# halismai/photobundle

Hardware: AMD Instinct MI355X
Metric: LM iters/sec + residuals/sec, 8-frame KITTI window, 50k pts, 5x5 patch (higher is better)
Workload: dtype f64; 1 GPU; configs[1]: 8-frame window, 50000 points/GPU, 5x5 patch, single level, dense visibility; image=1241x376 u8, observations=400000, sampler_precision=exact, channels=1, point_parameterisation=free world points (reference)

## Files before the change

__graft_entry__.py:

```python
import os
import subprocess
import sys

ROOT = os.path.dirname(os.path.abspath(__file__))
if ROOT not in sys.path:
    sys.path.insert(0, ROOT)


def build():
    env = dict(os.environ)
    subprocess.check_call(["make", "-s", "-C", os.path.join(ROOT, "photobundle_amd", "csrc")], env=env)
    subprocess.check_call(["make", "-s", "-C", os.path.join(ROOT, "photobundle_amd", "host")], env=env)
    subprocess.check_call(["make", "-s", "-C", os.path.join(ROOT, "oracle")], env=env)
    subprocess.check_call(["make", "-s", "-C", os.path.join(ROOT, "tests", "native")], env=env)
    import photobundle_amd
    from photobundle_amd import _lib
    _lib.lib()


def smoke():
    import numpy as np
    from oracle import oracle
    from photobundle_amd import synthetic
    from photobundle_amd.engine import Engine, default_solver_options

    p = synthetic.make_window(n_frames=4, n_points=300, radius=2, size=(120, 160), K=(200.0, 200.0, 80.0, 60.0))
    ref = oracle.solve(p, oracle.default_options(max_num_iterations=8))
    with Engine(120, 160, p.K, p.radius, p.n_frames, huber=p.huber, device=0) as e:
        e.load(p)
        res = e.solve(default_solver_options(max_num_iterations=8))
    assert len(res["iterations"]) == len(ref["iterations"])
    for a, b in zip(ref["iterations"], res["iterations"]):
        assert a["step_is_successful"] == b["step_is_successful"]
        assert abs(a["cost"] - b["cost"]) <= 1e-9 * abs(a["cost"]), (a["cost"], b["cost"])
    err = float(np.abs(res["cams"] - ref["cams"]).max())
    assert err <= 1e-5, err
    print("smoke ok: final cost %.6e (oracle %.6e), max pose diff %.3e" % (res["final_cost"], ref["final_cost"], err))


if __name__ == "__main__":
    build()
    if len(sys.argv) > 1 and sys.argv[1] == "smoke":
        smoke()
```

photobundle_amd/csrc/pba_solve.h:

```cpp
#pragma once

namespace pba {

__host__ __device__ inline int tri_index(int r) { return r * (r + 1) / 2; }
__host__ __device__ inline int packed_stride(int n) { return tri_index(n + 1) + 2 * n + 2; }

__host__ __device__ inline int solve_item_base(int j, int N1) { return (j - 1) * (N1 - 3 * j); }
inline int solve_table_words(int nf) { const int n = 6 * nf; return tri_index(n + 1) + (nf > 1 ? solve_item_base(nf, n + 1) : 0); }
inline void solve_tables(int nf, uint32_t* tab) {
  const int n = 6 * nf, N1 = n + 1, TRI = tri_index(N1);
  for (int r = 0; r < N1; ++r)
    for (int c = 0; c <= r; ++c) tab[tri_index(r) + c] = ((uint32_t)r << 16) | (uint32_t)c;
  for (int j = 1; j < nf; ++j)
    for (int r = 6 * j; r <= n; ++r) tab[TRI + solve_item_base(j, N1) + (r - 6 * j)] = (uint32_t)r | ((uint32_t)j << 16);
}

__device__ __forceinline__ int packed_dest(int e, int nf, int n_pairs) {
  const int n = 6 * nf, nT = 36 * n_pairs;
  if (e < nT) {
    const int pair = PBA_PARTIAL_T ? e % n_pairs : e / 36, k = PBA_PARTIAL_T ? e / n_pairs : e - 36 * pair, i = k / 6, j = k - 6 * i;
    int a = 0, rem = pair;
    while (rem >= nf - a) { rem -= nf - a; ++a; }
    const int b = a + rem;
    if (a == b && j < i) return -1;
// ... 250 lines not shown
}

__global__ __launch_bounds__(kSolveThreads) void k_solve_generic(SolveParams p_in) {
  SolveParams p = p_in;
  if (!solve_resolve(p)) return;
  extern __shared__ __attribute__((aligned(16))) char smem[];
  const int n = 6 * p.n_free;
  const int ld = n + 1;
  double* S = reinterpret_cast<double*>(smem);
  double* y = S + n * ld;
  double* sc = y + n;
  double* D2 = sc + n;
  double* gcs = D2 + n;
  double* gc = gcs + n;
  __shared__ int s_ok;
  const int tid = threadIdx.x;
  if (tid == 0) s_ok = 1;
  if (p.peer_world > 0 && !peer_wait_all(p.peer, p.peer_world, p.peer_flag, p.peer_seq, p.peer_timeout, p.peer_err, tid)) s_ok = 0;
  solve_prologue<kSolveThreads>(p, n, ld, S, y, sc, D2, gcs, gc, tid);
  const int tx = tid & 15, ty = tid >> 4;
  for (int j = 0; j < n; ++j) {
    const double d = S[j * ld + j];
    const double dj = (d > 0.0) ? sqrt(d) : 1.0;
    if (tid == 0 && (!(d > 0.0) || !isfinite(d))) s_ok = 0;
    __syncthreads();
    for (int r = j + tid; r < n; r += kSolveThreads) S[r * ld + j] = (r == j) ? dj : S[r * ld + j] / dj;
    __syncthreads();
    for (int r = j + 1 + ty; r < n; r += 16) {
      const double lrj = S[r * ld + j];
      for (int c = j + 1 + tx; c <= r; c += 16) S[r * ld + c] -= lrj * S[c * ld + j];
    }
    __syncthreads();
  }
  for (int j = 0; j < n; ++j) {
    if (tid == 0) y[j] /= S[j * ld + j];
    __syncthreads();
    const double yj = y[j];
    for (int r = j + 1 + tid; r < n; r += kSolveThreads) y[r] -= S[r * ld + j] * yj;
    __syncthreads();
  }
  for (int j = n - 1; j >= 0; --j) {
    if (tid == 0) y[j] /= S[j * ld + j];
    __syncthreads();
    const double yj = y[j];
    for (int r = tid; r < j; r += kSolveThreads) y[r] -= S[j * ld + r] * yj;
    __syncthreads();
  }
  solve_epilogue<kSolveThreads>(p, n, y, sc, D2, gcs, gc, s_ok != 0, tid);
}

constexpr int kSolveBlockedThreads = 256;
constexpr int kSolveWideThreads = 512;
constexpr int kSolveNarrowFree = 8;
__host__ __device__ inline size_t solve_blocked_smem_bytes(int n) {
  const size_t N1 = (size_t)n + 1;
  const size_t items = (size_t)(n / 6) * N1;
  return sizeof(double) * (N1 * N1 + 2 * 6 * N1 + 6 * N1 + 2) + sizeof(uint32_t) * items;
}

__device__ inline void cam_geom_scalar(const double cam6[6], double* cg) {
  const double wx = cam6[0], wy = cam6[1], wz = cam6[2];
  const double theta2 = wx * wx + wy * wy + wz * wz;
  const bool rod = theta2 > DBL_EPSILON;
#pragma unroll
  for (int k = 0; k < 6; ++k) cg[k] = cam6[k];
  double R[9], w3[3], ct, st;
  if (rod) {
    const double theta = sqrt(theta2);
    sincos_angle(theta, st, ct);
    const double ti = 1.0 / theta;
    const double ax = wx * ti, ay = wy * ti, az = wz * ti;
    const double oc = 1.0 - ct;
    w3[0] = ax; w3[1] = ay; w3[2] = az;
    R[0] = ct + ax * ax * oc;       R[1] = ax * ay * oc - az * st;  R[2] = ay * st + ax * az * oc;
    R[3] = az * st + ax * ay * oc;  R[4] = ct + ay * ay * oc;       R[5] = -ax * st + ay * az * oc;
    R[6] = -ay * st + ax * az * oc; R[7] = ax * st + ay * az * oc;  R[8] = ct + az * az * oc;
  } else {
    w3[0] = w3[1] = w3[2] = 0.0; ct = 1.0; st = 0.0;
    R[0] = 1; R[1] = -wz; R[2] = wy; R[3] = wz; R[4] = 1; R[5] = -wx; R[6] = -wy; R[7] = wx; R[8] = 1;
  }
#pragma unroll
  for (int k = 0; k < 3; ++k) cg[6 + k] = w3[k];
  cg[9] = ct; cg[10] = st;
#pragma unroll
  for (int k = 0; k < 9; ++k) cg[11 + k] = R[k];
  cg[20] = theta2;
  cg[21] = rod ? 1.0 : 0.0;
}

__device__ inline void cam_geom_finish(const double* cg, CamGeom* __restrict__ out, int c, uint32_t anchor_mask, int sub) {
  CamGeom& g = out[c];
  const bool rod = cg[21] != 0.0;
  if (sub < 3) { g.aa[sub] = cg[sub]; g.t[sub] = cg[3 + sub]; g.w[sub] = cg[6 + sub]; }
  if (sub == 3) {
    g.rodrigues = rod; g.is_free = slot_is_free(anchor_mask, c);
    g.free_index = slot_free_index(anchor_mask, c);
    g.pad = 0;
  }
  if (sub == 4) { g.ct = cg[9]; g.st = cg[10]; }
  const double* R = cg + 11;
  const int e9 = sub < 9 ? sub : 8;
  if (sub < 9) g.R[sub] = R[e9];
  const int s27 = sub < 27 ? sub : 26;
  double dRv;
  if (rod) {
    const int ei = e9 / 3, ej = e9 - 3 * ei;
    double acc = cg[ei] * cg[ej];
#pragma unroll
    for (int q = 0; q < 3; ++q) {
      const int d = (ej - q + 3) % 3;
      const double wo = cg[(d == 0) ? 0 : 3 - q - ej];
      const double wxqj = (d == 0) ? 0.0 : (d == 1 ? -wo : wo);
      acc += (R[3 * q + ei] - (ei == q ? 1.0 : 0.0)) * wxqj;
    }
    const double Bv = acc / cg[20];
    const int k = s27 / 9, ij = s27 - 9 * k, i = ij / 3, j = ij - 3 * i;
    const int lane0 = threadIdx.x & 32;
    const double b0 = __shfl(Bv, lane0 + k), b1 = __shfl(Bv, lane0 + 3 + k), b2 = __shfl(Bv, lane0 + 6 + k);
    const double x0 = (j == 0) ? 0.0 : (j == 1 ? -b2 : b1);
    const double x1 = (j == 0) ? b2 : (j == 1 ? 0.0 : -b0);
    const double x2 = (j == 0) ? -b1 : (j == 1 ? b0 : 0.0);
    double a3 = 0.0;
    a3 += R[3 * i] * x0; a3 += R[3 * i + 1] * x1; a3 += R[3 * i + 2] * x2;
    dRv = a3;
  } else {
    const int k = s27 / 9, m = s27 - 9 * k;
    const int i = m / 3, j = m - 3 * i;
    dRv = 0.0;
    if (i != j && i != k && j != k) dRv = ((j - i + 3) % 3 == 1) ? -1.0 : 1.0;
  }
  if (sub < 27) g.dR[sub] = dRv;
}

template <bool AGENT, int T>
__device__ __forceinline__ void solve_blocked(SolveParams& p, double* smem, int tid) {
  const int nf = p.n_free;
  const int n = 6 * nf;
  const int N1 = n + 1;
  const int ld = N1;
  double* A = smem;
  double* Wp = A + (size_t)N1 * ld;
  double* xs = Wp + 2 * (size_t)N1 * 6;
  double* sc = xs + N1;
  double* D2 = sc + N1;
  double* gcs = D2 + N1;
  double* gc = gcs + N1;
  double* live = gc + N1;
  uint32_t* items = reinterpret_cast<uint32_t*>(live + N1 + 1);
  __shared__ int s_ok;
  __shared__ double s_cams[6 * kMaxFrames];
  __shared__ int s_free[kMaxFrames];
  __shared__ double s_cg[kMaxFrames][32];
  __shared__ double s_stat[3];
  __shared__ double s_dyn[3];
  const int TRI = tri_index(N1);
  const int lane = tid & 63, wave = __builtin_amdgcn_readfirstlane(tid >> 6);
  unsigned long long ts[8] = {0, 0, 0, 0, 0, 0, 0, 0};
#define PBA_TS(k) do { if (PBA_PHASE_TIMING) ts[k] = __builtin_amdgcn_s_memtime(); } while (0)
  unsigned long long sec[8] = {0, 0, 0, 0, 0, 0, 0, 0}, sec_t = 0;
#define PBA_SEC(k) do { if (PBA_PHASE_TIMING) { const unsigned long long tn = __builtin_amdgcn_s_memtime(); if (k) sec[k] += tn - sec_t; sec_t = tn; } } while (0)
  PBA_TS(0);
  bool peer_ok = true;
  if (!AGENT && p.peer_world > 0) peer_ok = peer_wait_all(p.peer, p.peer_world, p.peer_flag, p.peer_seq, p.peer_timeout, p.peer_err, tid);
  constexpr int kPer = (T > 256) ? 9 : 5;
  double val[kPer];
#pragma unroll
  for (int u = 0; u < kPer; ++u) { const int t = tid + u * T; val[u] = (t < TRI) ? packed_load<AGENT>(p, t) : 0.0; }
  const double cam_v = (tid < 6 * p.n_frames) ? p.cams[tid] : 0.0;
  const int free_v = (tid < p.n_frames) ? p.geom[tid].free_index : -1;
  static_assert(T >= 6 * kMaxFrames, "one thread per reduced-system row");
  double du = 0.0, g = 0.0, s_old = 1.0, live_old = 0.0, cost_lin = 0.0, gn2_pts = 0.0;
  if (tid < n) {
    du = packed_load<AGENT>(p, TRI + n + tid);
    g = packed_load<AGENT>(p, TRI + tid);
    if (!p.init_scale) { s_old = p.sc[tid]; live_old = p.sc[n + tid]; }
  }
  if (tid == 0) { cost_lin = packed_load<AGENT>(p, TRI + 2 * n); gn2_pts = packed_load<AGENT>(p, TRI + 2 * n + 1); }
  uint32_t rc[kPer];
#pragma unroll
  for (int u = 0; u < kPer; ++u) { const int t = tid + u * T; rc[u] = (t < TRI) ? p.tab[t] : 0u; }
  const int n_items = (nf > 1) ? solve_item_base(nf, N1) : 0;
  constexpr int kItemsPer = (T > 256) ? 2 : 1;
  uint32_t itv[kItemsPer];
#pragma unroll
  for (int u = 0; u < kItemsPer; ++u) { const int t = tid + u * T; itv[u] = (t < n_items) ? p.tab[TRI + t] : 0u; }
#pragma unroll
  for (int u = 0; u < kItemsPer; ++u) { const int t = tid + u * T; if (t < n_items) items[t] = itv[u]; }
  if (tid < 6 * p.n_frames) s_cams[tid] = cam_v;
  if (tid < p.n_frames) s_free[tid] = free_v;
  if (tid < n) {
    const int i = tid;
    double s, lv;
    if (p.init_scale) { s = p.jacobi ? 1.0 / (1.0 + sqrt(du)) : 1.0; lv = du > 0.0 ? 1.0 : 0.0; p.sc[i] = s; p.sc[n + i] = lv; }
    else { s = s_old; lv = live_old; }
    sc[i] = s;
    live[i] = lv;
    D2[i] = fmin(fmax(s * s * du, p.min_diag), p.max_diag) / p.radius;
    gc[i] = g;
    gcs[i] = s * g;
  }
  if (tid == n) sc[n] = 1.0;
  if (tid == 0) s_ok = peer_ok ? 1 : 0;
  __syncthreads();
  PBA_TS(1);
#pragma unroll
  for (int u = 0; u < kPer; ++u) {
    const int t = tid + u * T;
    if (t >= TRI) continue;
    const int r = (int)(rc[u] >> 16), c = (int)(rc[u] & 0xffffu);
    double v = sc[c] * val[u] * sc[r];
    if (r == c) v = (r < n) ? v + D2[r] : 0.0;
    A[(size_t)r * ld + c] = v;
    if (r != c) A[(size_t)c * ld + r] = 0.0;
  }
  __syncthreads();
  if (p.S_dbg) {
    for (int k = tid; k < n * n; k += T) { const int r = k / n, c = k - r * n; p.S_dbg[k] = (r >= c) ? A[(size_t)r * ld + c] : A[(size_t)c * ld + r]; }
    for (int i = tid; i < n; i += T) p.rhs_dbg[i] = A[(size_t)n * ld + i];
    __syncthreads();
  }
  PBA_TS(2);
  constexpr int ROWS = (T > 256) ? 2 : 1;
  constexpr int NB = T - 64;
  if (wave == T / 64 - 1) {
    double q2[2] = {0.0, 0.0};
    double gmax = 0.0;
    for (int i = lane; i < n; i += 64) { gmax = fmax(gmax, fabs(gc[i])); q2[0] += gc[i] * gc[i]; }
    for (int i = lane; i < 6 * p.n_frames; i += 64) {
      const int fa = s_free[i / 6];
      if (fa < 0) continue;
      const double* lv = live + 6 * fa;
      if (lv[0] + lv[1] + lv[2] + lv[3] + lv[4] + lv[5] > 0.0) q2[1] += s_cams[i] * s_cams[i];
    }
    wave_sum_n<2>(q2);
    gmax = wave_max(gmax);
    if (lane == 0) { s_stat[0] = gmax; s_stat[1] = q2[0]; s_stat[2] = q2[1]; }
  }
  if (!(p.final_pass && !p.init_scale)) {
    if (wave == 0) {
      __builtin_amdgcn_s_setprio(3);
      double a[ROWS][6], w[ROWS][6];
      double Wd[21];
#pragma unroll
      for (int q = 0; q < ROWS; ++q) {
        const int r = lane + 64 * q;
#pragma unroll
        for (int m = 0; m < 6; ++m) { a[q][m] = A[(size_t)(r <= n ? r : n) * ld + m]; w[q][m] = 0.0; }
      }
#pragma unroll
      for (int i = 0; i < 6; ++i)
#pragma unroll
        for (int m = 0; m <= i; ++m) Wd[i * (i + 1) / 2 + m] = A[(size_t)i * ld + m];
      for (int k = 0; k < nf; ++k) {
        const int c0 = 6 * k;
        double Lt[21], rd[6];
        bool pd = true;
        PBA_SEC(0);
#pragma unroll
        for (int j = 0; j < 6; ++j) {
#pragma unroll
          for (int i = j; i < 6; ++i) {
            double v = Wd[i * (i + 1) / 2 + j];
#pragma unroll
            for (int m = 0; m < j; ++m) v = fma(-Wd[i * (i + 1) / 2 + m], Lt[j * (j + 1) / 2 + m], v);
            Wd[i * (i + 1) / 2 + j] = v;
          }
          const double d = Wd[j * (j + 1) / 2 + j];
          const bool ok = (d > 0.0) && isfinite(d);
          pd = pd && ok;
          rd[j] = fast_rcp(ok ? d : 1.0);
#pragma unroll
          for (int i = j + 1; i < 6; ++i) Lt[i * (i + 1) / 2 + j] = Wd[i * (i + 1) / 2 + j] * rd[j];
        }
        PBA_SEC(1);
        double* Wk = Wp + (size_t)(k & 1) * N1 * 6;
#pragma unroll
        for (int q = 0; q < ROWS; ++q) {
          const int r = lane + 64 * q;
          double l[6];
#pragma unroll
          for (int j = 0; j < 6; ++j) {
            double v = a[q][j];
#pragma unroll
            for (int m = 0; m < j; ++m) v = fma(-w[q][m], Lt[j * (j + 1) / 2 + m], v);
            w[q][j] = v;
            l[j] = v * rd[j];
          }
          if (r >= c0 && r <= n) {
#pragma unroll
            for (int m = 0; m < 6; ++m) { A[(size_t)r * ld + c0 + m] = l[m]; Wk[(size_t)r * 6 + m] = w[q][m]; }
            if (r == c0 && !pd) s_ok = 0;
          }
        }
        PBA_SEC(2);
        double Lb[36];
        const bool more = k + 1 < nf;
        if (more) {
          wave_lds_sync();
#pragma unroll
          for (int e = 0; e < 6; ++e)
#pragma unroll
            for (int m = 0; m < 6; ++m) Lb[6 * e + m] = A[(size_t)(c0 + 6 + e) * ld + c0 + m];
        }
        PBA_SEC(3);
        __syncthreads();
        PBA_SEC(4);
        if (!more) break;
#pragma unroll
        for (int q = 0; q < ROWS; ++q) {
          const int r = lane + 64 * q;
          const bool act = r >= c0 + 6 && r <= n;
          const double* arow = A + (size_t)(r <= n ? r : n) * ld + c0 + 6;
          double an[6];
#pragma unroll
          for (int e = 0; e < 6; ++e) an[e] = arow[e];
#pragma unroll
          for (int m = 0; m < 6; ++m)
#pragma unroll
            for (int e = 0; e < 6; ++e) an[e] = fma(-w[q][m], Lb[6 * e + m], an[e]);
          if (act && r < c0 + 12) {
#pragma unroll
            for (int e = 0; e < 6; ++e) A[(size_t)r * ld + c0 + 6 + e] = an[e];
          }
#pragma unroll
          for (int e = 0; e < 6; ++e) a[q][e] = an[e];
        }
        PBA_SEC(5);
        wave_lds_sync();
#pragma unroll
        for (int i = 0; i < 6; ++i)
#pragma unroll
          for (int m = 0; m <= i; ++m) Wd[i * (i + 1) / 2 + m] = A[(size_t)(c0 + 6 + i) * ld + c0 + 6 + m];
        if (PBA_PHASE_TIMING) { asm volatile("s_waitcnt lgkmcnt(0)" ::: "memory"); }
        PBA_SEC(6);
      }
      __builtin_amdgcn_s_setprio(0);
    } else {
      const int qb = tid - 64;
      for (int k = 0; k < nf; ++k) {
        __syncthreads();
        if (k + 2 >= nf) continue;
        const int c0 = 6 * k;
        const double* Wk = Wp + (size_t)(k & 1) * N1 * 6;
        for (int it = solve_item_base(k + 2, N1) + qb; it < n_items; it += NB) {
          const uint32_t wd = items[it];
          const int r = (int)(wd & 0xffffu), j = (int)(wd >> 16);
          double wr[6], lc[36], acc[6];
#pragma unroll
          for (int m = 0; m < 6; ++m) wr[m] = Wk[(size_t)r * 6 + m];
#pragma unroll
          for (int e = 0; e < 6; ++e)
#pragma unroll
            for (int m = 0; m < 6; ++m) lc[6 * e + m] = A[(size_t)(6 * j + e) * ld + c0 + m];
#pragma unroll
          for (int e = 0; e < 6; ++e) acc[e] = A[(size_t)r * ld + 6 * j + e];
#pragma unroll
          for (int e = 0; e < 6; ++e)
#pragma unroll
            for (int m = 0; m < 6; ++m) acc[e] = fma(-wr[m], lc[6 * e + m], acc[e]);
#pragma unroll
          for (int e = 0; e < 6; ++e) A[(size_t)r * ld + 6 * j + e] = acc[e];
        }
      }
    }
    for (int t = tid; t < n; t += T) {
      const int c0 = 6 * (t / 6);
#pragma unroll
      for (int m = 0; m < 6; ++m) if (c0 + m >= t) A[(size_t)t * ld + c0 + m] = 0.0;
    }
    __syncthreads();
    PBA_TS(3);
    if (wave == 0) {
      double z[ROWS];
#pragma unroll
      for (int q = 0; q < ROWS; ++q) { const int i = lane + 64 * q; z[q] = (i < n) ? A[(size_t)n * ld + i] : 0.0; }
      const double* Arow = A + (lane < n ? lane : 0);
      auto load_chunk = [&](int jb, double (&L6)[6][ROWS]) {
#pragma unroll
        for (int u = 0; u < 6; ++u)
#pragma unroll
          for (int q = 0; q < ROWS; ++q) L6[u][q] = Arow[(size_t)(jb + u) * ld + 64 * q];
      };
      auto apply_chunk = [&](int jb, const double (&L6)[6][ROWS]) {
#pragma unroll
        for (int u = 5; u >= 0; --u) {
          const int j = jb + u;
          const double zsrc = (ROWS == 2 && j >= 64) ? z[ROWS - 1] : z[0];
          const double xj = readlane_f64(zsrc, j & 63);
#pragma unroll
          for (int q = 0; q < ROWS; ++q) z[q] = fma(-L6[u][q], xj, z[q]);
        }
      };
      double LA[6][ROWS], LB[6][ROWS];
      int jb = n - 6;
      load_chunk(jb, LA);
      for (;;) {
        if (jb >= 6) load_chunk(jb - 6, LB);
        apply_chunk(jb, LA);
        jb -= 6;
        if (jb < 0) break;
        if (jb >= 6) load_chunk(jb - 6, LA);
        apply_chunk(jb, LB);
        jb -= 6;
        if (jb < 0) break;
      }
      double q2[2] = {0.0, 0.0};
      bool bad = false;
#pragma unroll
      for (int q = 0; q < ROWS; ++q) {
        const int i = lane + 64 * q;
        if (i < n) {
          xs[i] = z[q];
          q2[0] += 0.5 * z[q] * gcs[i] + 0.5 * D2[i] * z[q] * z[q];
          const double d = sc[i] * z[q];
          q2[1] += d * d;
          bad = bad || !isfinite(z[q]);
        }
      }
      wave_sum_n<2>(q2);
      const bool any_bad = __any(bad ? 1 : 0) != 0;
      if (lane == 0) { s_dyn[0] = q2[0]; s_dyn[1] = q2[1]; s_dyn[2] = any_bad ? 1.0 : 0.0; }
    }
    __syncthreads();
  } else {
    for (int i = tid; i < n; i += T) xs[i] = 0.0;
    if (tid == 0) { s_dyn[0] = 0.0; s_dyn[1] = 0.0; s_dyn[2] = 0.0; }
    __syncthreads();
  }
  PBA_TS(4);
  const bool chol_ok = s_ok != 0;
  const bool poisoned = !AGENT && p.peer_world > 0 && !peer_ok;
  const double qnan = __longlong_as_double(0x7ff8000000000000ll);
  if (tid < 6 * p.n_frames && !(p.final_pass && !p.init_scale)) {
    const int slot = tid / 6, k = tid % 6;
    const int fa = s_free[slot];
    double d = 0.0;
    if (fa >= 0) d = -sc[6 * fa + k] * xs[6 * fa + k];
    if (poisoned) d = qnan;
    p.delta_c[tid] = d;
    p.cams_cand[tid] = s_cams[tid] + d;
  }
  if (p.geom_cand) {
    if (wave == 1 && lane < p.n_frames) {
      const int c = lane;
      double cam6[6];
      const int fa = s_free[c];
#pragma unroll
      for (int k = 0; k < 6; ++k) cam6[k] = s_cams[6 * c + k] + (fa >= 0 ? -sc[6 * fa + k] * xs[6 * fa + k] : 0.0);
      cam_geom_scalar(cam6, s_cg[c]);
    }
  }
  if (tid == 0) {
    p.scal[kMccCams] = s_dyn[0]; p.scal[kStep2Cams] = s_dyn[1]; p.scal[kX2Cams] = s_stat[2];
    p.scal[kGmaxCams] = s_stat[0]; p.scal[kGnorm2Cams] = s_stat[1];
    p.scal[kSolveOk] = (chol_ok && s_dyn[2] == 0.0 && !poisoned) ? 1.0 : 0.0;
    p.scal[kCostLin] = poisoned ? qnan : cost_lin;
    p.scal[kGnorm2Pts] = gn2_pts;
  }
  PBA_TS(6);
  if (p.geom_cand) {
    __syncthreads();
    for (int c = tid / 32; c < p.n_frames; c += T / 32) cam_geom_finish(s_cg[c], p.geom_cand, c, p.anchor_mask, tid & 31);
  }
  PBA_TS(5);
  if (PBA_PHASE_TIMING && p.dbg && tid == 0)
    printf("solve_blocked n %d cycles: prologue %llu (loads + tables %llu, scatter %llu) factorisation %llu [block %llu rows %llu Lb %llu barrier %llu update %llu reload %llu] substitution %llu epilogue %llu (scalars %llu)\n",
           n, ts[2] - ts[0], ts[1] - ts[0], ts[2] - ts[1], ts[3] - ts[2], sec[1], sec[2], sec[3], sec[4], sec[5], sec[6], ts[4] - ts[3], ts[5] - ts[4], ts[6] - ts[4]);
#undef PBA_TS
#undef PBA_SEC
}

template <int T>
__global__ __launch_bounds__(T) void k_solve_blocked(SolveParams p_in) {
  SolveParams p = p_in;
  if (!solve_resolve(p)) return;
  extern __shared__ __attribute__((aligned(16))) char smem[];
  solve_blocked<false, T>(p, reinterpret_cast<double*>(smem), threadIdx.x);
}

struct ReduceFinalParams {
  ReduceParams rp;
  const LmState* lm; int32_t enq_cur, final_pass;
  const double* block_cost_alt; const int32_t* block_fail_alt;
  int32_t sys_stores;
  unsigned int* ticket;
  double* peer_own; int32_t peer_flag; unsigned long long peer_seq;
};
__global__ __launch_bounds__(kReduceThreads) void k_reduce_final(ReduceFinalParams fp) {
  ReduceParams rp = fp.rp;
  const bool skip = fp.lm && ((fp.lm->done && !fp.final_pass) || (fp.final_pass && !lm_final_pass_needed(fp.lm)));
  __shared__ double s_red[kReduceThreads / kReduceEntries][kReduceEntries + 1];
  __shared__ int s_f[16];
  if (!skip) {
    if (fp.lm && fp.lm->cur != fp.enq_cur) { rp.block_cost = fp.block_cost_alt; rp.block_fail = fp.block_fail_alt; }
    if (fp.sys_stores) reduce_partials<2>(rp, s_red, s_f, (int)blockIdx.x, (int)gridDim.x);
    else reduce_partials<0>(rp, s_red, s_f, (int)blockIdx.x, (int)gridDim.x);
  }
  if (fp.peer_flag >= 0) {
    asm volatile("s_waitcnt vmcnt(0)" ::: "memory");
    __syncthreads();
    if (threadIdx.x == 0) {
      const unsigned t = __hip_atomic_fetch_add(fp.ticket, 1u, __ATOMIC_ACQ_REL, __HIP_MEMORY_SCOPE_AGENT);
      if (t == gridDim.x - 1) {
        *fp.ticket = 0;
        __hip_atomic_store(reinterpret_cast<unsigned long long*>(fp.peer_own) + fp.peer_flag, fp.peer_seq, __ATOMIC_RELEASE, __HIP_MEMORY_SCOPE_SYSTEM);
// ... 96 lines not shown
```

photobundle_amd/csrc/pba_kernels.h:

```cpp
#pragma once
#include "pba_device.h"

#include <cfloat>
#include <climits>
#include <type_traits>

#ifndef PBA_PHASE_TIMING
#define PBA_PHASE_TIMING 0
#endif

#ifndef PBA_SAMPLE_WAVES_PER_SIMD
#define PBA_SAMPLE_WAVES_PER_SIMD 4
#endif
#ifndef PBA_SAMPLE_WAVES_LARGE
#define PBA_SAMPLE_WAVES_LARGE 2
#endif
#ifndef PBA_EXPERIMENT_SKIP_IRREGULAR
#define PBA_EXPERIMENT_SKIP_IRREGULAR 0
#endif
#ifndef PBA_WALK_ROWWISE
#define PBA_WALK_ROWWISE 0
#endif

#ifndef PBA_REC_SC1
// ... 1882 lines not shown
}

template <class RL>
__device__ __forceinline__ void schur_body(SchurParams& p, char* smem, const int tid, const int part, const int n_parts, RL* rl,
                                           const CamGeom* geom_res, const bool has_tile) {
  constexpr bool RES = !std::is_void<RL>::value;
  double* s_obs = reinterpret_cast<double*>(smem);
  static_assert(1024 + kTile * 9 <= kTile * kObsStride && kMaxFrames * sizeof(CamGeom) <= 1024 * sizeof(double), "aliasing fits");
  double* s_vg = s_obs + 1024;
  double* s_tot = s_obs + 1024 + kTile * 9;
  uint16_t* s_ptl = reinterpret_cast<uint16_t*>(s_obs + 1024 + 2 * kTile * 9);
  static_assert(1024 + 2 * kTile * 9 + kTile / 4 <= kTile * kObsStride, "point totals fit before W | Y");
  double* s_red = s_obs + kTile * kObsStride;
  int8_t* s_lane_of = reinterpret_cast<int8_t*>(s_red + kTile);

  const int nf = p.n_free;
  const int n_groups = kTile / p.n_pairs;
  const int grp = tid / p.n_pairs;
  const int pair = tid - grp * p.n_pairs;
  const bool owner = grp < n_groups;
  int pa = 0, pb = 0;
  {
    int a = 0, rem = pair;
    while (rem >= nf - a) { rem -= nf - a; ++a; }
    pa = a; pb = a + rem;
  }
  double acc[36];
#pragma unroll
  for (int k = 0; k < 36; ++k) acc[k] = 0.0;
  constexpr int kCamVals = 33;
  constexpr int kCamAcc = (kCamVals * (kMaxFrames - 1) + kTile - 1) / kTile;
  double acc_cam[kCamAcc];
#pragma unroll
  for (int u = 0; u < kCamAcc; ++u) acc_cam[u] = 0.0;
  double gmax = 0.0, gn2 = 0.0;
  int fail = 0;
  static_assert(sizeof(CamGeom) % 8 == 0, "CamGeom is copied as 8-byte words");
  constexpr int kGeomRegs = 4;
  const int n_geom_words = p.n_frames * (int)(sizeof(CamGeom) / 8);
  unsigned long long greg[kGeomRegs];
#pragma unroll
  for (int u = 0; u < kGeomRegs; ++u) {
    const int k = tid + u * kTile;
    greg[u] = (!RES && k < n_geom_words) ? reinterpret_cast<const unsigned long long*>(p.geom)[k] : 0ull;
  }

  if (tid < kCamVals) s_red[tid] = 0.0;
  static_assert(kCamVals <= kTile, "zero row fits s_red");
  unsigned long long tph[8] = {0, 0, 0, 0, 0, 0, 0, 0};
  unsigned long long tlast = p.dbg ? __builtin_amdgcn_s_memtime() : 0;
  const unsigned long long t_rt0 = p.dbg ? __builtin_amdgcn_s_memrealtime() : 0;
#define PBA_TICK(k) do { if (p.dbg) { const unsigned long long tn = __builtin_amdgcn_s_memtime(); tph[k] += tn - tlast; tlast = tn; } } while (0)
  int4 ti_next = make_int4(0, 0, 0, 0);
  int nx_pt = 0, nx_slot = 0, nx_l0 = 0, nx_cnt = 0;
  double nx_x[3] = {0.0, 0.0, 0.0};
  if constexpr (RES) {
    if (has_tile) { ti_next = rl->ti; nx_pt = rl->pt; nx_slot = rl->slot; nx_l0 = rl->l0; nx_cnt = rl->cnt; nx_x[0] = rl->X[0]; nx_x[1] = rl->X[1]; nx_x[2] = rl->X[2]; }
  } else {
    ti_next = p.tile_info[min(part, p.n_tiles - 1)];
    {
      const int2 r = p.lane_rec[(size_t)min(part, p.n_tiles - 1) * kTile + tid];
      nx_pt = r.x; nx_slot = r.y & 0xff; nx_l0 = (r.y >> 8) & 0xff; nx_cnt = (r.y >> 16) & 0xff;
    }
    if (tid < ti_next.y) {
      nx_x[0] = p.xyz[3 * (size_t)nx_pt]; nx_x[1] = p.xyz[3 * (size_t)nx_pt + 1]; nx_x[2] = p.xyz[3 * (size_t)nx_pt + 2];
    }
  }
  for (int tile = part; RES ? (tile == part) : (tile < p.n_tiles); tile += n_parts) {
    const int4 ti = ti_next;
    if constexpr (!RES) ti_next = p.tile_info[min(tile + n_parts, p.n_tiles - 1)];
    const int cur_pt = nx_pt, cur_slot = nx_slot, cur_l0 = nx_l0, cur_cnt = nx_cnt;
    const double cur_x[3] = {nx_x[0], nx_x[1], nx_x[2]};
    const int o0 = ti.x, n_here = ti.y, pt0 = ti.z, n_pts = ti.w;
    const bool active = tid < n_here;
    const int obs = o0 + tid;

    for (int k = tid; k < kMaxFrames * kTile / 4; k += kTile) reinterpret_cast<uint32_t*>(s_lane_of)[k] = 0x80808080u;
    const CamGeom* s_geom = RES ? geom_res : reinterpret_cast<const CamGeom*>(s_obs);
    if constexpr (!RES) {
#pragma unroll
    for (int u = 0; u < kGeomRegs; ++u) {
      const int k = tid + u * kTile;
      if (k < n_geom_words) reinterpret_cast<unsigned long long*>(s_obs)[k] = greg[u];
    }
    }
    if constexpr (!RES) {
      constexpr int kTail = (kMaxFrames * (int)(sizeof(CamGeom) / 8) + kTile - 1) / kTile - kGeomRegs;
      unsigned long long gt[kTail];
#pragma unroll
      for (int u = 0; u < kTail; ++u) {
        const int k = tid + (kGeomRegs + u) * kTile;
        gt[u] = (k < n_geom_words) ? reinterpret_cast<const unsigned long long*>(p.geom)[k] : 0ull;
      }
#pragma unroll
      for (int u = 0; u < kTail; ++u) {
        const int k = tid + (kGeomRegs + u) * kTile;
        if (k < n_geom_words) reinterpret_cast<unsigned long long*>(s_obs)[k] = gt[u];
      }
    }
    lds_barrier();
    PBA_TICK(0);

    int pt = 0, fa = -1, l0 = 0, l1 = 0;
    double Ac[2][6], Ap[2][3], M[3] = {0, 0, 0}, b[2] = {0, 0};
    double MAp[2][3];
    double s_pt[3] = {1.0, 1.0, 1.0};
    if (active) {
      pt = cur_pt;
      const int slot = cur_slot;
      l0 = cur_l0; l1 = l0 + cur_cnt;
      if constexpr (RES) { if (!p.init_scale) { s_pt[0] = rl->sp[0]; s_pt[1] = rl->sp[1]; s_pt[2] = rl->sp[2]; } }
      else if (!p.init_scale) { s_pt[0] = p.sp[3 * (size_t)pt]; s_pt[1] = p.sp[3 * (size_t)pt + 1]; s_pt[2] = p.sp[3 * (size_t)pt + 2]; }
      const CamGeom& g = s_geom[slot];
      fa = g.free_index;
      const double prm[3] = {cur_x[0], cur_x[1], cur_x[2]};
      double X[3], qd[3];
      point_world(p.rays, pt, prm, X, qd);
      double xw[3];
      transform_point(g, X, xw);
      projection_jacobians(g, X, xw, p.fx, p.fy, Ac, Ap);
      point_jacobian(p.rays, qd, Ap);
      if constexpr (RES) { M[0] = rl->rec[0]; M[1] = rl->rec[1]; M[2] = rl->rec[2]; b[0] = rl->rec[3]; b[1] = rl->rec[4]; }
      else {
      M[0] = p.rec[0 * p.rec_stride + obs]; M[1] = p.rec[1 * p.rec_stride + obs]; M[2] = p.rec[2 * p.rec_stride + obs];
      b[0] = p.rec[3 * p.rec_stride + obs]; b[1] = p.rec[4 * p.rec_stride + obs];
      }
#pragma unroll
      for (int k = 0; k < 3; ++k) { MAp[0][k] = M[0] * Ap[0][k] + M[1] * Ap[1][k]; MAp[1][k] = M[1] * Ap[0][k] + M[2] * Ap[1][k]; }
      double* vg = s_vg + tid * 9;
      vg[0] = Ap[0][0] * MAp[0][0] + Ap[1][0] * MAp[1][0];
      vg[1] = Ap[0][0] * MAp[0][1] + Ap[1][0] * MAp[1][1];
      vg[2] = Ap[0][0] * MAp[0][2] + Ap[1][0] * MAp[1][2];
      vg[3] = Ap[0][1] * MAp[0][1] + Ap[1][1] * MAp[1][1];
      vg[4] = Ap[0][1] * MAp[0][2] + Ap[1][1] * MAp[1][2];
      vg[5] = Ap[0][2] * MAp[0][2] + Ap[1][2] * MAp[1][2];
#pragma unroll
      for (int k = 0; k < 3; ++k) vg[6 + k] = -(Ap[0][k] * b[0] + Ap[1][k] * b[1]);
      if (fa >= 0) s_lane_of[fa * kTile + (pt - pt0)] = (int8_t)tid;
      if (tid == l0) s_ptl[pt - pt0] = (uint16_t)(l0 | ((l1 - l0) << 8));
    }
    lds_barrier();
    PBA_TICK(1);

    double V[6] = {0, 0, 0, 0, 0, 0}, gp[3] = {0, 0, 0};
    for (int k = tid; k < 9 * n_pts; k += kTile) {
      const int q = k / 9, c = k - 9 * q;
      const unsigned lc = s_ptl[q];
      const int ql0 = (int)(lc & 0xffu), qcnt = (int)(lc >> 8);
      const double* src = s_vg + ql0 * 9 + c;
      double a = 0.0;
      double x[8];
#pragma unroll
      for (int l = 0; l < 8; ++l) x[l] = src[9 * (l < qcnt ? l : qcnt - 1)];
#pragma unroll
      for (int l = 0; l < 8; ++l) a += (l < qcnt) ? x[l] : 0.0;
      if (qcnt > 8) {
#pragma unroll
        for (int l = 8; l < kMaxFrames; ++l) x[l - 8] = src[9 * (l < qcnt ? l : qcnt - 1)];
#pragma unroll
        for (int l = 8; l < kMaxFrames; ++l) a += (l < qcnt) ? x[l - 8] : 0.0;
      }
      s_tot[k] = a;
    }
    lds_barrier();
    if (active) {
      const double* tot = s_tot + (pt - pt0) * 9;
#pragma unroll
      for (int k = 0; k < 6; ++k) V[k] = tot[k];
#pragma unroll
      for (int k = 0; k < 3; ++k) gp[k] = tot[6 + k];
    }
    lds_barrier();
    PBA_TICK(2);
    const bool grad_only = p.final_pass != 0 && !p.init_scale;
    double Pm[6] = {0, 0, 0, 0, 0, 0};
    if (active && grad_only) {
      if (tid == l0) {
#pragma unroll
        for (int k = 0; k < 3; ++k) { gmax = fmax(gmax, fabs(gp[k])); gn2 += gp[k] * gp[k]; }
      }
    } else if (active) {
      const bool head = (tid == l0);
      double s[3];
      const double vd[3] = {V[0], V[3], V[5]};
      if (p.init_scale) {
#pragma unroll
        for (int k = 0; k < 3; ++k) s[k] = p.jacobi ? 1.0 / (1.0 + sqrt(vd[k])) : 1.0;
        if constexpr (RES) { rl->sp[0] = s[0]; rl->sp[1] = s[1]; rl->sp[2] = s[2]; }
        else if (head) { p.sp[3 * (size_t)pt] = s[0]; p.sp[3 * (size_t)pt + 1] = s[1]; p.sp[3 * (size_t)pt + 2] = s[2]; }
      } else {
#pragma unroll
        for (int k = 0; k < 3; ++k) s[k] = s_pt[k];
      }
      double D2[3];
#pragma unroll
      for (int k = 0; k < 3; ++k) D2[k] = fmin(fmax(s[k] * s[k] * vd[k], p.min_diag), p.max_diag) * p.inv_radius;
      const double a00 = s[0] * s[0] * V[0] + D2[0], a01 = s[0] * s[1] * V[1], a02 = s[0] * s[2] * V[2];
      const double a11 = s[1] * s[1] * V[3] + D2[1], a12 = s[1] * s[2] * V[4], a22 = s[2] * s[2] * V[5] + D2[2];
      bool pd = a00 > 0.0;
      const double i00 = fast_rsqrt(a00);
      const double l10 = a01 * i00, l20 = a02 * i00;
      const double d1 = a11 - l10 * l10;
      pd = pd && d1 > 0.0;
      const double i11 = fast_rsqrt(d1);
      const double l21 = (a12 - l20 * l10) * i11;
      const double d2 = a22 - l20 * l20 - l21 * l21;
      pd = pd && d2 > 0.0;
      const double i22 = fast_rsqrt(d2);
      if (pd) {
        const double i10 = -l10 * i00 * i11;
        const double i21 = -l21 * i11 * i22;
        const double i20 = -(l20 * i00 + l21 * i10) * i22;
        const double v00 = i00 * i00 + i10 * i10 + i20 * i20;
        const double v01 = i10 * i11 + i20 * i21;
        const double v02 = i20 * i22;
        const double v11 = i11 * i11 + i21 * i21;
        const double v12 = i21 * i22;
        const double v22 = i22 * i22;
        Pm[0] = s[0] * s[0] * v00; Pm[1] = s[0] * s[1] * v01; Pm[2] = s[0] * s[2] * v02;
        Pm[3] = s[1] * s[1] * v11; Pm[4] = s[1] * s[2] * v12; Pm[5] = s[2] * s[2] * v22;
      } else if (head) {
        fail = 1;
      }
      if constexpr (RES) {
#pragma unroll
        for (int k = 0; k < 6; ++k) rl->pr[k] = Pm[k];
#pragma unroll
        for (int k = 0; k < 3; ++k) { rl->pr[6 + k] = gp[k]; rl->pr[9 + k] = D2[k]; }
      }
      if (head) {
        if constexpr (!RES) {
        double* pr = p.ptrec + 12 * (size_t)pt;
#pragma unroll
        for (int k = 0; k < 6; ++k) pr[k] = Pm[k];
#pragma unroll
        for (int k = 0; k < 3; ++k) { pr[6 + k] = gp[k]; pr[9 + k] = D2[k]; }
        }
#pragma unroll
        for (int k = 0; k < 3; ++k) { gmax = fmax(gmax, fabs(gp[k])); gn2 += gp[k] * gp[k]; }
      }
    }
    if (active && fa >= 0 && grad_only) {
      double* so = s_obs + tid * kObsStride;
#pragma unroll
      for (int j = 0; j < 6; ++j) so[27 + j] = -(Ac[0][j] * b[0] + Ac[1][j] * b[1]);
    } else if (active && fa >= 0) {
      double* so = s_obs + tid * kObsStride;
      const double Pg[3] = {Pm[0] * gp[0] + Pm[1] * gp[1] + Pm[2] * gp[2], Pm[1] * gp[0] + Pm[3] * gp[1] + Pm[4] * gp[2],
                            Pm[2] * gp[0] + Pm[4] * gp[1] + Pm[5] * gp[2]};
      const double bq0 = b[0] + (MAp[0][0] * Pg[0] + MAp[0][1] * Pg[1] + MAp[0][2] * Pg[2]);
      const double bq1 = b[1] + (MAp[1][0] * Pg[0] + MAp[1][1] * Pg[1] + MAp[1][2] * Pg[2]);
#pragma unroll
      for (int j = 0; j < 6; ++j) {
        so[27 + j] = -(Ac[0][j] * b[0] + Ac[1][j] * b[1]);
        so[21 + j] = -(Ac[0][j] * bq0 + Ac[1][j] * bq1);
      }
      double MAc[2][6];
#pragma unroll
      for (int j = 0; j < 6; ++j) { MAc[0][j] = M[0] * Ac[0][j] + M[1] * Ac[1][j]; MAc[1][j] = M[1] * Ac[0][j] + M[2] * Ac[1][j]; }
#pragma unroll
      for (int i = 0; i < 6; ++i)
#pragma unroll
        for (int j = i; j < 6; ++j) so[sym6(i, j)] = Ac[0][i] * MAc[0][j] + Ac[1][i] * MAc[1][j];
    }
    lds_barrier();
    PBA_TICK(3);
    if (!RES && tile + n_parts < p.n_tiles) {
      const int2 r = p.lane_rec[(size_t)(tile + n_parts) * kTile + tid];
      nx_pt = r.x; nx_slot = r.y & 0xff; nx_l0 = (r.y >> 8) & 0xff; nx_cnt = (r.y >> 16) & 0xff;
    }

#pragma unroll
    for (int u = 0; u < kCamAcc; ++u) {
      const int e = tid + u * kTile;
      if (e < kCamVals * nf) {
        const int a = e / kCamVals, v = e - a * kCamVals;
        if (grad_only && v < 27) continue;
        for (int q0 = 0; q0 < n_pts; q0 += 16) {
          const int4 l4 = *reinterpret_cast<const int4*>(s_lane_of + a * kTile + q0);
          const int lw[4] = {l4.x, l4.y, l4.z, l4.w};
#pragma unroll
          for (int h = 0; h < 2; ++h) {
            if (q0 + 8 * h >= n_pts) continue;
            int off[8];
#pragma unroll
            for (int k = 0; k < 8; ++k) off[k] = (int)((lw[2 * h + (k >> 2)] >> (8 * (k & 3))) & 0xff) * kObsStride + v;
            double x[8];
#pragma unroll
            for (int k = 0; k < 8; ++k) x[k] = s_obs[off[k]];
#pragma unroll
            for (int k = 0; k < 8; ++k) acc_cam[u] += x[k];
          }
        }
      }
    }
    lds_barrier();
    PBA_TICK(4);
    if (!RES && tile + n_parts < p.n_tiles && tid < ti_next.y) {
      nx_x[0] = p.xyz[3 * (size_t)nx_pt]; nx_x[1] = p.xyz[3 * (size_t)nx_pt + 1]; nx_x[2] = p.xyz[3 * (size_t)nx_pt + 2];
    }
    if (grad_only) continue;
    if (active && fa >= 0) {
      double* so = s_obs + tid * kObsStride;
#pragma unroll
      for (int k = 0; k < 3; ++k) { so[k] = Ac[0][k]; so[3 + k] = Ac[1][k]; }
      so[6] = Ac[0][3]; so[7] = Ac[0][5]; so[8] = Ac[1][4]; so[9] = Ac[1][5];
#pragma unroll
      for (int r = 0; r < 2; ++r) {
        so[10 + 3 * r] = MAp[r][0]; so[11 + 3 * r] = MAp[r][1]; so[12 + 3 * r] = MAp[r][2];
        so[16 + 3 * r] = MAp[r][0] * Pm[0] + MAp[r][1] * Pm[1] + MAp[r][2] * Pm[2];
        so[17 + 3 * r] = MAp[r][0] * Pm[1] + MAp[r][1] * Pm[3] + MAp[r][2] * Pm[4];
        so[18 + 3 * r] = MAp[r][0] * Pm[2] + MAp[r][1] * Pm[4] + MAp[r][2] * Pm[5];
      }
    }
    lds_barrier();
    PBA_TICK(5);

    if (owner) {
      const int8_t* la_row = s_lane_of + pa * kTile;
      const int8_t* lb_row = s_lane_of + pb * kTile;
      for (int q = grp; q < n_pts; q += n_groups) {
        const int la = la_row[q], lb = lb_row[q];
        if (la < 0 || lb < 0) continue;
        const double* Fa = s_obs + la * kObsStride;
        const double* Fb = s_obs + lb * kObsStride;
        double aa[10], qa[6], ab[10], mb[6];
#pragma unroll
        for (int k = 0; k < 10; ++k) { aa[k] = Fa[k]; ab[k] = Fb[k]; }
#pragma unroll
        for (int k = 0; k < 6; ++k) { qa[k] = Fa[16 + k]; mb[k] = Fb[10 + k]; }
        double N[2][2];
#pragma unroll
        for (int r = 0; r < 2; ++r)
#pragma unroll
          for (int t = 0; t < 2; ++t) N[r][t] = fma(qa[3 * r + 2], mb[3 * t + 2], fma(qa[3 * r + 1], mb[3 * t + 1], qa[3 * r] * mb[3 * t]));
        double Z[2][6];
#pragma unroll
        for (int r = 0; r < 2; ++r) {
#pragma unroll
          for (int j = 0; j < 3; ++j) Z[r][j] = fma(N[r][1], ab[3 + j], N[r][0] * ab[j]);
          Z[r][3] = N[r][0] * ab[6];
          Z[r][4] = N[r][1] * ab[8];
          Z[r][5] = fma(N[r][1], ab[9], N[r][0] * ab[7]);
        }
#pragma unroll
        for (int j = 0; j < 6; ++j) {
#pragma unroll
          for (int i = 0; i < 3; ++i) acc[6 * i + j] = fma(-aa[3 + i], Z[1][j], fma(-aa[i], Z[0][j], acc[6 * i + j]));
          acc[18 + j] = fma(-aa[6], Z[0][j], acc[18 + j]);
          acc[24 + j] = fma(-aa[8], Z[1][j], acc[24 + j]);
// ... 271 lines not shown
```

Measured before the change: 9904 LM iters/s of the one 50000-point window (50k points per GPU: weak scaling; not multiplied by N).

## Add compile-time levers to restructure reduced-camera solve kernel phases

Adds a PBA_SOLVE_LEVERS bitmask, with all levers on by default, that changes four parts of the blocked camera solve. The scatter prologue preloads scale and damping values into registers before writing. The reciprocal is computed before the positive-definite select. Loading of the Lb block moves after the barrier so the pre-barrier wave sync can be dropped. The step-norm sums move from the solving wave to wave 2 after the barrier, with the scalar writes reassigned to thread 128. The goal is to shorten the critical path of the single-wave substitution and factorisation at the cost of an extra LDS read pass.

New measurement: 9989 LM iters/s of the one 50000-point window (50k points per GPU: weak scaling; not multiplied by N) (median of 3 runs). About the same (+0.9%).

```diff
diff --git a/__graft_entry__.py b/__graft_entry__.py
--- a/__graft_entry__.py
+++ b/__graft_entry__.py
@@ -9,7 +9,7 @@
 
 def build():
     env = dict(os.environ)
-    subprocess.check_call(["make", "-s", "-C", os.path.join(ROOT, "photobundle_amd", "csrc")], env=env)
+    subprocess.check_call(["make", "-s", "-j2", "-C", os.path.join(ROOT, "photobundle_amd", "csrc"), "all", "ab"], env=env)
     subprocess.check_call(["make", "-s", "-C", os.path.join(ROOT, "photobundle_amd", "host")], env=env)
     subprocess.check_call(["make", "-s", "-C", os.path.join(ROOT, "oracle")], env=env)
     subprocess.check_call(["make", "-s", "-C", os.path.join(ROOT, "tests", "native")], env=env)
diff --git a/photobundle_amd/csrc/pba_solve.h b/photobundle_amd/csrc/pba_solve.h
--- a/photobundle_amd/csrc/pba_solve.h
+++ b/photobundle_amd/csrc/pba_solve.h
@@ -326,6 +326,11 @@
 constexpr int kSolveBlockedThreads = 256;
 constexpr int kSolveWideThreads = 512;
 constexpr int kSolveNarrowFree = 8;
+#ifndef PBA_SOLVE_LEVERS
+#define PBA_SOLVE_LEVERS 15
+#endif
+constexpr bool kLevSumsOff = (PBA_SOLVE_LEVERS & 1) != 0, kLevRcpSelect = (PBA_SOLVE_LEVERS & 2) != 0, kLevLbBehind = (PBA_SOLVE_LEVERS & 4) != 0,
+               kLevScatter2 = (PBA_SOLVE_LEVERS & 8) != 0;
 __host__ __device__ inline size_t solve_blocked_smem_bytes(int n) {
   const size_t N1 = (size_t)n + 1;
   const size_t items = (size_t)(n / 6) * N1;
@@ -429,6 +434,7 @@
   __shared__ double s_dyn[3];
   const int TRI = tri_index(N1);
   const int lane = tid & 63, wave = __builtin_amdgcn_readfirstlane(tid >> 6);
+  const int scal_tid = kLevSumsOff ? 128 : 0;
   unsigned long long ts[8] = {0, 0, 0, 0, 0, 0, 0, 0};
 #define PBA_TS(k) do { if (PBA_PHASE_TIMING) ts[k] = __builtin_amdgcn_s_memtime(); } while (0)
   unsigned long long sec[8] = {0, 0, 0, 0, 0, 0, 0, 0}, sec_t = 0;
@@ -449,7 +455,7 @@
     g = packed_load<AGENT>(p, TRI + tid);
     if (!p.init_scale) { s_old = p.sc[tid]; live_old = p.sc[n + tid]; }
   }
-  if (tid == 0) { cost_lin = packed_load<AGENT>(p, TRI + 2 * n); gn2_pts = packed_load<AGENT>(p, TRI + 2 * n + 1); }
+  if (tid == scal_tid) { cost_lin = packed_load<AGENT>(p, TRI + 2 * n); gn2_pts = packed_load<AGENT>(p, TRI + 2 * n + 1); }
   uint32_t rc[kPer];
 #pragma unroll
   for (int u = 0; u < kPer; ++u) { const int t = tid + u * T; rc[u] = (t < TRI) ? p.tab[t] : 0u; }
@@ -477,15 +483,34 @@
   if (tid == 0) s_ok = peer_ok ? 1 : 0;
   __syncthreads();
   PBA_TS(1);
-#pragma unroll
-  for (int u = 0; u < kPer; ++u) {
-    const int t = tid + u * T;
-    if (t >= TRI) continue;
-    const int r = (int)(rc[u] >> 16), c = (int)(rc[u] & 0xffffu);
-    double v = sc[c] * val[u] * sc[r];
-    if (r == c) v = (r < n) ? v + D2[r] : 0.0;
-    A[(size_t)r * ld + c] = v;
-    if (r != c) A[(size_t)c * ld + r] = 0.0;
+  if (kLevScatter2) {
+    double scc[kPer], scr[kPer], dd[kPer];
+#pragma unroll
+    for (int u = 0; u < kPer; ++u) {
+      const int r = (int)(rc[u] >> 16), c = (int)(rc[u] & 0xffffu);
+      scc[u] = sc[c]; scr[u] = sc[r]; dd[u] = D2[r < n ? r : 0];
+    }
+#pragma unroll
+    for (int u = 0; u < kPer; ++u) {
+      const int t = tid + u * T;
+      if (t >= TRI) continue;
+      const int r = (int)(rc[u] >> 16), c = (int)(rc[u] & 0xffffu);
+      double v = scc[u] * val[u] * scr[u];
+      if (r == c) v = (r < n) ? v + dd[u] : 0.0;
+      A[(size_t)r * ld + c] = v;
+      if (r != c) A[(size_t)c * ld + r] = 0.0;
+    }
+  } else {
+#pragma unroll
+    for (int u = 0; u < kPer; ++u) {
+      const int t = tid + u * T;
+      if (t >= TRI) continue;
+      const int r = (int)(rc[u] >> 16), c = (int)(rc[u] & 0xffffu);
+      double v = sc[c] * val[u] * sc[r];
+      if (r == c) v = (r < n) ? v + D2[r] : 0.0;
+      A[(size_t)r * ld + c] = v;
+      if (r != c) A[(size_t)c * ld + r] = 0.0;
+    }
   }
   __syncthreads();
   if (p.S_dbg) {
@@ -542,7 +567,8 @@
           const double d = Wd[j * (j + 1) / 2 + j];
           const bool ok = (d > 0.0) && isfinite(d);
           pd = pd && ok;
-          rd[j] = fast_rcp(ok ? d : 1.0);
+          if (kLevRcpSelect) { const double y = fast_rcp(d); rd[j] = ok ? y : 1.0; }
+          else rd[j] = fast_rcp(ok ? d : 1.0);
 #pragma unroll
           for (int i = j + 1; i < 6; ++i) Lt[i * (i + 1) / 2 + j] = Wd[i * (i + 1) / 2 + j] * rd[j];
         }
@@ -569,7 +595,7 @@
         PBA_SEC(2);
         double Lb[36];
         const bool more = k + 1 < nf;
-        if (more) {
+        if (more && !kLevLbBehind) {
           wave_lds_sync();
 #pragma unroll
           for (int e = 0; e < 6; ++e)
@@ -580,6 +606,12 @@
         __syncthreads();
         PBA_SEC(4);
         if (!more) break;
+        if (kLevLbBehind) {
+#pragma unroll
+          for (int e = 0; e < 6; ++e)
+#pragma unroll
+            for (int m = 0; m < 6; ++m) Lb[6 * e + m] = A[(size_t)(c0 + 6 + e) * ld + c0 + m];
+        }
 #pragma unroll
         for (int q = 0; q < ROWS; ++q) {
           const int r = lane + 64 * q;
@@ -678,24 +710,47 @@
         jb -= 6;
         if (jb < 0) break;
       }
+      if (kLevSumsOff) {
+#pragma unroll
+        for (int q = 0; q < ROWS; ++q) { const int i = lane + 64 * q; if (i < n) xs[i] = z[q]; }
+      } else {
+        double q2[2] = {0.0, 0.0};
+        bool bad = false;
+#pragma unroll
+        for (int q = 0; q < ROWS; ++q) {
+          const int i = lane + 64 * q;
+          if (i < n) {
+            xs[i] = z[q];
+            q2[0] += 0.5 * z[q] * gcs[i] + 0.5 * D2[i] * z[q] * z[q];
+            const double d = sc[i] * z[q];
+            q2[1] += d * d;
+            bad = bad || !isfinite(z[q]);
+          }
+        }
+        wave_sum_n<2>(q2);
+        const bool any_bad = __any(bad ? 1 : 0) != 0;
+        if (lane == 0) { s_dyn[0] = q2[0]; s_dyn[1] = q2[1]; s_dyn[2] = any_bad ? 1.0 : 0.0; }
+      }
+    }
+    __syncthreads();
+    if (kLevSumsOff && wave == 2) {
       double q2[2] = {0.0, 0.0};
       bool bad = false;
 #pragma unroll
       for (int q = 0; q < ROWS; ++q) {
         const int i = lane + 64 * q;
         if (i < n) {
-          xs[i] = z[q];
-          q2[0] += 0.5 * z[q] * gcs[i] + 0.5 * D2[i] * z[q] * z[q];
-          const double d = sc[i] * z[q];
+          const double zq = xs[i];
+          q2[0] += 0.5 * zq * gcs[i] + 0.5 * D2[i] * zq * zq;
+          const double d = sc[i] * zq;
           q2[1] += d * d;
-          bad = bad || !isfinite(z[q]);
+          bad = bad || !isfinite(zq);
         }
       }
       wave_sum_n<2>(q2);
       const bool any_bad = __any(bad ? 1 : 0) != 0;
       if (lane == 0) { s_dyn[0] = q2[0]; s_dyn[1] = q2[1]; s_dyn[2] = any_bad ? 1.0 : 0.0; }
     }
-    __syncthreads();
   } else {
     for (int i = tid; i < n; i += T) xs[i] = 0.0;
     if (tid == 0) { s_dyn[0] = 0.0; s_dyn[1] = 0.0; s_dyn[2] = 0.0; }
@@ -724,7 +779,7 @@
       cam_geom_scalar(cam6, s_cg[c]);
     }
   }
-  if (tid == 0) {
+  if (tid == scal_tid) {
     p.scal[kMccCams] = s_dyn[0]; p.scal[kStep2Cams] = s_dyn[1]; p.scal[kX2Cams] = s_stat[2];
     p.scal[kGmaxCams] = s_stat[0]; p.scal[kGnorm2Cams] = s_stat[1];
     p.scal[kSolveOk] = (chol_ok && s_dyn[2] == 0.0 && !poisoned) ? 1.0 : 0.0;
```

## Hoist per-tile global loads before barrier and unroll point-reduction loop by two

Applied to the files above, without the earlier changes.

Moves the next-tile tile_info load, the per-point scale load and the five rec loads so they issue before the first LDS barrier, letting their latency overlap the geometry copy. tile_info is now loaded into vector registers and made uniform with readfirstlane later, and lane metadata is kept packed and unpacked only when used. The LDS point-reduction loop now processes two elements per iteration to expose more independent loads. Register pressure rises, and the asm barriers on tid are there to steer scalar versus vector placement.

Result: no change. 9852 LM iters/s of the one 50000-point window (50k points per GPU: weak scaling; not multiplied by N) before, 9831 LM iters/s of the one 50000-point window (50k points per GPU: weak scaling; not multiplied by N) after, median of 2 (-0.2%).

```diff
diff --git a/photobundle_amd/csrc/pba_kernels.h b/photobundle_amd/csrc/pba_kernels.h
--- a/photobundle_amd/csrc/pba_kernels.h
+++ b/photobundle_amd/csrc/pba_kernels.h
@@ -1958,15 +1958,15 @@
   const unsigned long long t_rt0 = p.dbg ? __builtin_amdgcn_s_memrealtime() : 0;
 #define PBA_TICK(k) do { if (p.dbg) { const unsigned long long tn = __builtin_amdgcn_s_memtime(); tph[k] += tn - tlast; tlast = tn; } } while (0)
   int4 ti_next = make_int4(0, 0, 0, 0);
-  int nx_pt = 0, nx_slot = 0, nx_l0 = 0, nx_cnt = 0;
+  int nx_pt = 0, nx_meta = 0;
   double nx_x[3] = {0.0, 0.0, 0.0};
   if constexpr (RES) {
-    if (has_tile) { ti_next = rl->ti; nx_pt = rl->pt; nx_slot = rl->slot; nx_l0 = rl->l0; nx_cnt = rl->cnt; nx_x[0] = rl->X[0]; nx_x[1] = rl->X[1]; nx_x[2] = rl->X[2]; }
+    if (has_tile) { ti_next = rl->ti; nx_pt = rl->pt; nx_x[0] = rl->X[0]; nx_x[1] = rl->X[1]; nx_x[2] = rl->X[2]; }
   } else {
     ti_next = p.tile_info[min(part, p.n_tiles - 1)];
     {
       const int2 r = p.lane_rec[(size_t)min(part, p.n_tiles - 1) * kTile + tid];
-      nx_pt = r.x; nx_slot = r.y & 0xff; nx_l0 = (r.y >> 8) & 0xff; nx_cnt = (r.y >> 16) & 0xff;
+      nx_pt = r.x; nx_meta = r.y;
     }
     if (tid < ti_next.y) {
       nx_x[0] = p.xyz[3 * (size_t)nx_pt]; nx_x[1] = p.xyz[3 * (size_t)nx_pt + 1]; nx_x[2] = p.xyz[3 * (size_t)nx_pt + 2];
@@ -1974,8 +1974,11 @@
   }
   for (int tile = part; RES ? (tile == part) : (tile < p.n_tiles); tile += n_parts) {
     const int4 ti = ti_next;
-    if constexpr (!RES) ti_next = p.tile_info[min(tile + n_parts, p.n_tiles - 1)];
-    const int cur_pt = nx_pt, cur_slot = nx_slot, cur_l0 = nx_l0, cur_cnt = nx_cnt;
+    int tl = tid;
+    asm volatile("" : "+v"(tl));
+    const int cur_pt = nx_pt;
+    int cur_slot = nx_meta & 0xff, cur_l0 = (nx_meta >> 8) & 0xff, cur_cnt = (nx_meta >> 16) & 0xff;
+    if constexpr (RES) { if (has_tile) { cur_slot = rl->slot; cur_l0 = rl->l0; cur_cnt = rl->cnt; } }
     const double cur_x[3] = {nx_x[0], nx_x[1], nx_x[2]};
     const int o0 = ti.x, n_here = ti.y, pt0 = ti.z, n_pts = ti.w;
     const bool active = tid < n_here;
@@ -1995,14 +1998,25 @@
       unsigned long long gt[kTail];
 #pragma unroll
       for (int u = 0; u < kTail; ++u) {
-        const int k = tid + (kGeomRegs + u) * kTile;
+        const int k = tl + (kGeomRegs + u) * kTile;
         gt[u] = (k < n_geom_words) ? reinterpret_cast<const unsigned long long*>(p.geom)[k] : 0ull;
       }
 #pragma unroll
       for (int u = 0; u < kTail; ++u) {
-        const int k = tid + (kGeomRegs + u) * kTile;
+        const int k = tl + (kGeomRegs + u) * kTile;
         if (k < n_geom_words) reinterpret_cast<unsigned long long*>(s_obs)[k] = gt[u];
       }
+    }
+    int4 ti_v = make_int4(0, 0, 0, 0);
+    double rec_r[5] = {0, 0, 0, 0, 0}, sp_r[3] = {1.0, 1.0, 1.0};
+    if constexpr (!RES) {
+      int nxt = min(tile + n_parts, p.n_tiles - 1);
+      asm("" : "+v"(nxt));
+      ti_v = p.tile_info[nxt];
+      if (!p.init_scale) { sp_r[0] = p.sp[3 * (size_t)cur_pt]; sp_r[1] = p.sp[3 * (size_t)cur_pt + 1]; sp_r[2] = p.sp[3 * (size_t)cur_pt + 2]; }
+      const double* rec_o = p.rec + (active ? obs : o0);
+#pragma unroll
+      for (int k = 0; k < 5; ++k) rec_r[k] = rec_o[k * p.rec_stride];
     }
     lds_barrier();
     PBA_TICK(0);
@@ -2016,7 +2030,7 @@
       const int slot = cur_slot;
       l0 = cur_l0; l1 = l0 + cur_cnt;
       if constexpr (RES) { if (!p.init_scale) { s_pt[0] = rl->sp[0]; s_pt[1] = rl->sp[1]; s_pt[2] = rl->sp[2]; } }
-      else if (!p.init_scale) { s_pt[0] = p.sp[3 * (size_t)pt]; s_pt[1] = p.sp[3 * (size_t)pt + 1]; s_pt[2] = p.sp[3 * (size_t)pt + 2]; }
+      else if (!p.init_scale) { s_pt[0] = sp_r[0]; s_pt[1] = sp_r[1]; s_pt[2] = sp_r[2]; }
       const CamGeom& g = s_geom[slot];
       fa = g.free_index;
       const double prm[3] = {cur_x[0], cur_x[1], cur_x[2]};
@@ -2027,10 +2041,7 @@
       projection_jacobians(g, X, xw, p.fx, p.fy, Ac, Ap);
       point_jacobian(p.rays, qd, Ap);
       if constexpr (RES) { M[0] = rl->rec[0]; M[1] = rl->rec[1]; M[2] = rl->rec[2]; b[0] = rl->rec[3]; b[1] = rl->rec[4]; }
-      else {
-      M[0] = p.rec[0 * p.rec_stride + obs]; M[1] = p.rec[1 * p.rec_stride + obs]; M[2] = p.rec[2 * p.rec_stride + obs];
-      b[0] = p.rec[3 * p.rec_stride + obs]; b[1] = p.rec[4 * p.rec_stride + obs];
-      }
+      else { M[0] = rec_r[0]; M[1] = rec_r[1]; M[2] = rec_r[2]; b[0] = rec_r[3]; b[1] = rec_r[4]; }
 #pragma unroll
       for (int k = 0; k < 3; ++k) { MAp[0][k] = M[0] * Ap[0][k] + M[1] * Ap[1][k]; MAp[1][k] = M[1] * Ap[0][k] + M[2] * Ap[1][k]; }
       double* vg = s_vg + tid * 9;
@@ -2049,24 +2060,40 @@
     PBA_TICK(1);
 
     double V[6] = {0, 0, 0, 0, 0, 0}, gp[3] = {0, 0, 0};
-    for (int k = tid; k < 9 * n_pts; k += kTile) {
-      const int q = k / 9, c = k - 9 * q;
-      const unsigned lc = s_ptl[q];
-      const int ql0 = (int)(lc & 0xffu), qcnt = (int)(lc >> 8);
-      const double* src = s_vg + ql0 * 9 + c;
-      double a = 0.0;
-      double x[8];
-#pragma unroll
-      for (int l = 0; l < 8; ++l) x[l] = src[9 * (l < qcnt ? l : qcnt - 1)];
-#pragma unroll
-      for (int l = 0; l < 8; ++l) a += (l < qcnt) ? x[l] : 0.0;
-      if (qcnt > 8) {
-#pragma unroll
-        for (int l = 8; l < kMaxFrames; ++l) x[l - 8] = src[9 * (l < qcnt ? l : qcnt - 1)];
-#pragma unroll
-        for (int l = 8; l < kMaxFrames; ++l) a += (l < qcnt) ? x[l - 8] : 0.0;
-      }
-      s_tot[k] = a;
+    for (int k = tl; k < 9 * n_pts; k += 2 * kTile) {
+      const bool two = k + kTile < 9 * n_pts;
+      const int kk[2] = {k, two ? k + kTile : k};
+      const double* src[2];
+      int qcnt[2];
+#pragma unroll
+      for (int j = 0; j < 2; ++j) {
+        const int q = kk[j] / 9, c = kk[j] - 9 * q;
+        const unsigned lc = s_ptl[q];
+        qcnt[j] = (int)(lc >> 8);
+        src[j] = s_vg + (int)(lc & 0xffu) * 9 + c;
+      }
+      double a[2] = {0.0, 0.0};
+      double x[2][8];
+#pragma unroll
+      for (int j = 0; j < 2; ++j)
+#pragma unroll
+        for (int l = 0; l < 8; ++l) x[j][l] = src[j][9 * (l < qcnt[j] ? l : qcnt[j] - 1)];
+#pragma unroll
+      for (int l = 0; l < 8; ++l)
+#pragma unroll
+        for (int j = 0; j < 2; ++j) a[j] += (l < qcnt[j]) ? x[j][l] : 0.0;
+      if (qcnt[0] > 8 || qcnt[1] > 8) {
+#pragma unroll
+        for (int j = 0; j < 2; ++j)
+#pragma unroll
+          for (int l = 8; l < kMaxFrames; ++l) x[j][l - 8] = src[j][9 * (l < qcnt[j] ? l : qcnt[j] - 1)];
+#pragma unroll
+        for (int l = 8; l < kMaxFrames; ++l)
+#pragma unroll
+          for (int j = 0; j < 2; ++j) a[j] += (l < qcnt[j]) ? x[j][l - 8] : 0.0;
+      }
+      s_tot[k] = a[0];
+      if (two) s_tot[k + kTile] = a[1];
     }
     lds_barrier();
     if (active) {
@@ -2172,8 +2199,8 @@
     lds_barrier();
     PBA_TICK(3);
     if (!RES && tile + n_parts < p.n_tiles) {
-      const int2 r = p.lane_rec[(size_t)(tile + n_parts) * kTile + tid];
-      nx_pt = r.x; nx_slot = r.y & 0xff; nx_l0 = (r.y >> 8) & 0xff; nx_cnt = (r.y >> 16) & 0xff;
+      const int2 r = p.lane_rec[(size_t)(tile + n_parts) * kTile + tl];
+      nx_pt = r.x; nx_meta = r.y;
     }
 
 #pragma unroll
@@ -2202,6 +2229,10 @@
     }
     lds_barrier();
     PBA_TICK(4);
+    if constexpr (!RES) {
+      ti_next = make_int4(__builtin_amdgcn_readfirstlane(ti_v.x), __builtin_amdgcn_readfirstlane(ti_v.y),
+                          __builtin_amdgcn_readfirstlane(ti_v.z), __builtin_amdgcn_readfirstlane(ti_v.w));
+    }
     if (!RES && tile + n_parts < p.n_tiles && tid < ti_next.y) {
       nx_x[0] = p.xyz[3 * (size_t)nx_pt]; nx_x[1] = p.xyz[3 * (size_t)nx_pt + 1]; nx_x[2] = p.xyz[3 * (size_t)nx_pt + 2];
     }
```
